# SandroMartens/DBGSOM

Measured on NVIDIA B200. Metric: training samples/sec/epoch, higher is better.
Workload: dtype f16 tensor cores (tcgen05) + f64 re-score / f64 update / f64 smoothing

## Files before the change

dbgsom_b200/csrc/bmu_tc.cu:

```cuda
#include <cuda.h>

#include <cstdio>
#include <cstdlib>

#include "common.cuh"

namespace dbgsom {

namespace {

constexpr int BM = 128;
constexpr int BK = 64;
constexpr int UMMA_K = 16;
constexpr int A_TILE_BYTES = BM * BK * 2;
constexpr int EPI_WARP0 = 4;
constexpr int EPI_SUBS = 4;
constexpr int EPI_WARPS = 4 * EPI_SUBS;
constexpr int EPI_THREADS = EPI_WARPS * 32;
constexpr int TC_THREADS = (EPI_WARP0 + EPI_WARPS) * 32;
constexpr int KSUB = 4;
constexpr int MAX_RES_KB = 4;
constexpr int kFlagMaxCols = 4096;
constexpr int kFlagChunkBytes = kFlagMaxCols / 32 * BM * 4;

// ... 190 lines not shown
}
__device__ __forceinline__ int4 lds_i4(uint32_t a) {
  int4 v;
  asm volatile("ld.shared.v4.s32 {%0,%1,%2,%3}, [%4];" : "=r"(v.x), "=r"(v.y), "=r"(v.z), "=r"(v.w) : "r"(a));
  return v;
}
__device__ __forceinline__ void sts_f1(uint32_t a, float v) { asm volatile("st.shared.f32 [%0], %1;" ::"r"(a), "f"(v) : "memory"); }
__device__ __forceinline__ void sts_i1(uint32_t a, int v) { asm volatile("st.shared.s32 [%0], %1;" ::"r"(a), "r"(v) : "memory"); }
__device__ __forceinline__ bool pair_after(float va, int ja, float vb, int jb) {
  return va > vb || (va == vb && ja > jb);
}

struct EpiConst {
  const int32_t* proto_of_col;
  uint32_t pstride, mpad;
  int any_order;
};
constexpr uint32_t kTabIdxOffset = 128 * 4 * 4 * 4;

__device__ __noinline__ float2 slow_offer(float s, int col, uint32_t val_addr, uint32_t const_addr) {
  const EpiConst* ec;
  {
    uint64_t g;
    asm volatile("cvta.shared.u64 %0, %1;" : "=l"(g) : "l"((uint64_t)const_addr));
    ec = reinterpret_cast<const EpiConst*>(g);
  }
  const uint32_t idx_addr = val_addr + kTabIdxOffset;
  const int j = ec->pstride ? (int)(((uint32_t)col * ec->pstride) % ec->mpad) : ec->proto_of_col[col];
  const float4 v4 = lds_f4(val_addr);
  const int4 j4 = lds_i4(idx_addr);
  float v0 = v4.x, v1 = v4.y, v2 = v4.z, v3 = v4.w;
  int c0 = j4.x, c1 = j4.y, c2 = j4.z, c3 = j4.w;
  int w = 0;
  float wv = v0;
  int wc = c0;
  if (pair_after(v1, c1, wv, wc)) { w = 1; wv = v1; wc = c1; }
  if (pair_after(v2, c2, wv, wc)) { w = 2; wv = v2; wc = c2; }
  if (pair_after(v3, c3, wv, wc)) { w = 3; wv = v3; wc = c3; }
  const bool replace = pair_after(wv, wc, s, j);
  const float out = replace ? wv : s;
  if (replace) {
    sts_f1(val_addr + 4 * w, s);
    sts_i1(idx_addr + 4 * w, j);
    if (w == 0) v0 = s;
    if (w == 1) v1 = s;
    if (w == 2) v2 = s;
    if (w == 3) v3 = s;
  }
  float g = fmaxf(fmaxf(v0, v1), fmaxf(v2, v3));
  if (!ec->any_order && g < 3.0e38f) g = nextafterf(g, __int_as_float(0x7f800000));
  return make_float2(g, out);
}

template <int NPASS, int BN, int RES_KB, int AKB, bool PAIRS = false, int EXTRA_BYTES = 0>
struct Cfg {
  static constexpr bool ATM = AKB > 0;
  static constexpr bool XRES = RES_KB > 0;
  static constexpr bool ASTREAM = !XRES && !ATM;
  static constexpr int NA = NPASS == 3 ? 2 : 1;
  static constexpr int B_TILE_BYTES = BN * BK * 2;
  static_assert(!PAIRS || ASTREAM, "PAIRS is the streamed form");
  static constexpr int STAGE_BYTES = NA * (PAIRS ? B_TILE_BYTES / 2 : B_TILE_BYTES) + (ASTREAM ? NA * A_TILE_BYTES : 0);
  static_assert(!ATM || (RES_KB == 0 && B_TILE_BYTES <= A_TILE_BYTES), "TMEM-resident A shares the ring: BN <= 128");
  static constexpr int A_COLS = AKB * NA * (BK / 2);
  static constexpr int NACC = ATM ? ((512 - A_COLS) / BN > 4 ? 4 : (512 - A_COLS) / BN) : (PAIRS && BN == 128 ? 4 : 2);
  static_assert(NACC >= 2, "need two accumulator buffers");
  static constexpr int RES_BYTES = RES_KB * NA * A_TILE_BYTES;
  static constexpr int RING_BYTES = BM * EPI_SUBS * KSUB * 8 + BM * 4 + BM * EPI_SUBS * 16;
  static constexpr int MISC_BYTES = 1024;
  static constexpr int WN_SMEM_FLOATS = ATM ? 4096 : 0;
  static constexpr int WN_BYTES = WN_SMEM_FLOATS * 4;
  static constexpr int SMEM_BUDGET = 227 * 1024 - 1024;
  static constexpr int STAGE_UNIT = ATM ? (STAGE_BYTES > A_TILE_BYTES ? STAGE_BYTES : A_TILE_BYTES) : STAGE_BYTES;
  static constexpr int STAGES_RAW = (SMEM_BUDGET - RES_BYTES - RING_BYTES - MISC_BYTES - WN_BYTES - EXTRA_BYTES) / STAGE_UNIT;
  static constexpr int STAGES = STAGES_RAW > (ATM ? 12 : 8) ? (ATM ? 12 : 8) : STAGES_RAW;
  static constexpr int RING_STAGE_BYTES = STAGES * STAGE_UNIT;
  static constexpr int SMEM_BYTES = RES_BYTES + RING_STAGE_BYTES + RING_BYTES + MISC_BYTES + WN_BYTES + EXTRA_BYTES + 1024;
  static constexpr int TMEM_COLS = ATM ? 512 : NACC * BN;
  static_assert(STAGES >= 2, "not enough shared memory for a pipeline");
};

struct Barriers {
  uint64_t full[16], empty[16];
  uint64_t a_full, a_empty;
  uint64_t tmem_full[4], tmem_empty[4];
  uint32_t tmem_base;
  EpiConst epi;
};

constexpr float kTileBoundFloor = 0.125f;
template <int NPASS, int NB, int BN, int RES_KB, int AKB, int CL, bool PAIR = false, int SEL = 0, bool TB = false,
          int SGT = 0>
__global__ void __launch_bounds__(TC_THREADS, 1)
    bmu_cand_tensor_kernel(const __grid_constant__ CUtensorMap map_xh, const __grid_constant__ CUtensorMap map_xl,
                           const __grid_constant__ CUtensorMap map_wh, const __grid_constant__ CUtensorMap map_wl,
                           const __grid_constant__ CUtensorMap map_wb, const float* __restrict__ bias_scale,
                           int64_t N, int KB, int NT, const float* __restrict__ wnorm,
                           const int32_t* __restrict__ proto_of_col, int pstride, int ties_any,
                           const float* __restrict__ xnorm16,
                           const float* __restrict__ wmax, float bound_coef, float acc_coef,
                           int32_t* __restrict__ idx_out, int32_t* __restrict__ cand_idx,
                           uint8_t* __restrict__ cand_count, const int32_t* __restrict__ row_perm,
                           unsigned long long* __restrict__ tile_mask,
                           int fg_shift, unsigned long long* __restrict__ sel_stats,
                           const float* __restrict__ tile_bound) {
  static_assert(!TB || (NB == 1 && SEL == 0 && BN % 128 == 0), "tile bounds: classic one-winner search, 128-column granules");
  using C = Cfg<NPASS, BN, RES_KB, AKB, PAIR && AKB == 0 && RES_KB == 0, SEL == 1 ? kFlagChunkBytes : 0>;
  static_assert(SEL == 0 || (PAIR && AKB > 0 && NB == 1 && NPASS == (SEL == 1 ? 1 : 3)),
                "selective search: CTA pairs, sample tile in tensor memory, one winner");
  constexpr bool ATM = C::ATM;
  static_assert(!PAIR || (CL == 2 && (ATM || C::ASTREAM)), "the CTA-pair form needs a cluster of two; sample tile in tensor memory or streamed");
  constexpr int B_PART_BYTES = PAIR ? C::B_TILE_BYTES / 2 : C::B_TILE_BYTES;
  constexpr bool SEGM = PAIR && C::ASTREAM && BN == 128;
  constexpr int SEG = 4;
  constexpr bool SEGT = SGT > 0;
  static_assert(!SEGT || (PAIR && C::ASTREAM && BN == 256 && C::NACC == 2 && SEL == 0), "tensor-memory sums: streamed pair form, 256 columns");
  static_assert(!SEGM || BN / 32 == EPI_SUBS, "segmented accumulation: one chunk per epilogue warp and tile");
  constexpr bool PAIR_ATM = PAIR && ATM;
  constexpr int SLOT_BYTES = PAIR_ATM ? A_TILE_BYTES : C::STAGE_BYTES;
  constexpr int NSLOT = PAIR_ATM ? (C::RING_STAGE_BYTES / A_TILE_BYTES > 16 ? 16 : C::RING_STAGE_BYTES / A_TILE_BYTES)
                                 : C::STAGES;
  static_assert(!PAIR_ATM || C::NA * B_PART_BYTES <= SLOT_BYTES, "a prototype k-block of the pair form must fit a slot");
  constexpr int NACC = C::NACC;
  constexpr bool XRES = C::XRES;
  constexpr bool ASTREAM = C::ASTREAM;
  extern __shared__ uint8_t smem_raw[];
  uint8_t* smem = reinterpret_cast<uint8_t*>((reinterpret_cast<uintptr_t>(smem_raw) + 1023) & ~uintptr_t(1023));
  uint8_t* res_a = smem;
  uint8_t* stages = smem + C::RES_BYTES;
  float* wn_smem = reinterpret_cast<float*>(stages + C::RING_STAGE_BYTES);
  uint8_t* ring = stages + C::RING_STAGE_BYTES + C::WN_BYTES;
  Barriers* bars = reinterpret_cast<Barriers*>(ring + C::RING_BYTES);
  float* chunk_min = reinterpret_cast<float*>(ring + C::RING_BYTES + C::MISC_BYTES);
  float* tab_val = reinterpret_cast<float*>(ring);
  int* tab_idx = reinterpret_cast<int*>(ring + BM * EPI_SUBS * KSUB * 4);
  float* row_min = reinterpret_cast<float*>(ring + BM * EPI_SUBS * KSUB * 8);
  float4* sub_state = reinterpret_cast<float4*>(ring + BM * EPI_SUBS * KSUB * 8 + BM * 4);

  const int warp = threadIdx.x >> 5;
  const int lane = threadIdx.x & 31;
  const int64_t n_row_tiles = ceil_div<int64_t>(N, BM);
  const uint32_t cl_rank = CL > 1 ? cluster_ctarank() : 0u;
  const int64_t n_clusters = gridDim.x / CL;
  const int64_t cluster_id = blockIdx.x / CL;
  const int64_t n_iters = ceil_div<int64_t>(n_row_tiles, n_clusters * CL);
  constexpr uint16_t cl_mask = (uint16_t)((1u << CL) - 1u);
  auto tile_of = [&](int64_t it) { return (it * n_clusters + cluster_id) * CL + cl_rank; };
  const int64_t n_pairs = ceil_div<int64_t>(n_row_tiles, 2);
  auto pair_of = [&](int64_t it) { return it * n_clusters + cluster_id; };
  auto sel_mask = [&](int64_t it) -> unsigned long long {
    const int64_t pr = pair_of(it);
    return (SEL == 2 && pr < n_pairs) ? tile_mask[pr] : 0ull;
  };

  if (warp == 0 && lane == 0) {
    tma_prefetch_desc(&map_xh);
    tma_prefetch_desc(&map_wh);
    if (NPASS == 3) {
      tma_prefetch_desc(&map_xl);
      tma_prefetch_desc(&map_wl);
    }
  }
  if (warp == 1 && lane == 0) {
    for (int s = 0; s < NSLOT; ++s) {
      mbar_init(&bars->full[s], PAIR ? 2 : 1);
      mbar_init(&bars->empty[s], PAIR ? 1 : CL);
    }
    mbar_init(&bars->a_full, 1);
    mbar_init(&bars->a_empty, 1);
    for (int b = 0; b < NACC; ++b) {
      mbar_init(&bars->tmem_full[b], 1);
      mbar_init(&bars->tmem_empty[b], PAIR ? 2 * EPI_WARPS : EPI_THREADS);
    }
    asm volatile("fence.mbarrier_init.release.cluster;" ::: "memory");
  }
  if (warp == 2) {
    if (PAIR) {
      asm volatile("tcgen05.alloc.cta_group::2.sync.aligned.shared::cta.b32 [%0], %1;" ::"r"(smem_u32(&bars->tmem_base)),
                   "r"((uint32_t)C::TMEM_COLS)
                   : "memory");
      asm volatile("tcgen05.relinquish_alloc_permit.cta_group::2.sync.aligned;" ::: "memory");
    } else {
      asm volatile("tcgen05.alloc.cta_group::1.sync.aligned.shared::cta.b32 [%0], %1;" ::"r"(smem_u32(&bars->tmem_base)),
                   "r"((uint32_t)C::TMEM_COLS)
                   : "memory");
      asm volatile("tcgen05.relinquish_alloc_permit.cta_group::1.sync.aligned;" ::: "memory");
    }
  }
// ... 22 lines not shown
      unsigned long long pmask_next = SEL == 2 ? sel_mask(0) : 0ull;
      for (int64_t it = 0; it < n_iters; ++it) {
        const int row0 = (int)(tile_of(it) * BM);
        const unsigned long long pmask_it = pmask_next;
        if (SEL == 2) pmask_next = it + 1 < n_iters ? sel_mask(it + 1) : 0ull;
        if (XRES) {
          mbar_wait(&bars->a_empty, a_phase ^ 1);
          mbar_expect_tx(&bars->a_full, (uint32_t)(KB * C::NA * A_TILE_BYTES));
          for (int kb = 0; kb < KB; ++kb) {
            tma_load_2d(res_a + (kb * C::NA + 0) * A_TILE_BYTES, &map_xh, &bars->a_full, kb * BK, row0);
            if (NPASS == 3) tma_load_2d(res_a + (kb * C::NA + 1) * A_TILE_BYTES, &map_xl, &bars->a_full, kb * BK, row0);
          }
          a_phase ^= 1;
        }
        if (ATM) {
          for (int kb = 0; kb < KB; ++kb) {
            if (PAIR) {
              for (int h = 0; h < C::NA; ++h) {
                mbar_wait(&bars->empty[stage], phase ^ 1);
                const uint32_t lead_full = mapa_u32(smem_u32(&bars->full[stage]), 0);
                if (cl_rank == 0) mbar_expect_tx(&bars->full[stage], (uint32_t)(2 * A_TILE_BYTES));
                else mbar_arrive_cluster(lead_full);
                tma_load_2d_pair(stages + stage * SLOT_BYTES, h == 0 ? &map_xh : &map_xl, lead_full, kb * BK, row0);
                if (++stage == NSLOT) {
                  stage = 0;
                  phase ^= 1;
                }
              }
              continue;
            }
            mbar_wait(&bars->empty[stage], phase ^ 1);
            uint8_t* st = stages + stage * C::STAGE_BYTES;
            mbar_expect_tx(&bars->full[stage], (uint32_t)(C::NA * A_TILE_BYTES));
            tma_load_2d(st, &map_xh, &bars->full[stage], kb * BK, row0);
            if (NPASS == 3) tma_load_2d(st + A_TILE_BYTES, &map_xl, &bars->full[stage], kb * BK, row0);
            if (++stage == C::STAGES) {
              stage = 0;
              phase ^= 1;
            }
          }
        }
        unsigned long long selm = pmask_it;
        const int n_sel = SEL == 2 ? __popcll(selm) : NT;
        if (SEL == 2 && cl_rank == 0 && pair_of(it) < n_pairs) {
          sel_tiles += (unsigned)n_sel;
          ++sel_pairs;
        }
        for (int ti = 0; ti < n_sel; ++ti) {
          int nt = ti;
          if (SEL == 2) {
            nt = __ffsll((long long)selm) - 1;
            selm &= selm - 1;
          }
          for (int kb = 0; kb < KB; ++kb) {
            mbar_wait(&bars->empty[stage], phase ^ 1);
            uint8_t* st = stages + stage * SLOT_BYTES;
            if (PAIR) {
              const uint32_t lead_full = mapa_u32(smem_u32(&bars->full[stage]), 0);
              if (cl_rank == 0) mbar_expect_tx(&bars->full[stage], (uint32_t)(2 * (C::NA * B_PART_BYTES + (ASTREAM ? C::NA * A_TILE_BYTES : 0))));
              else mbar_arrive_cluster(lead_full);
              const int prow = nt * BN + (int)cl_rank * (BN / 2);
              tma_load_2d_pair(st, &map_wh, lead_full, kb * BK, prow);
              if (NPASS == 3) tma_load_2d_pair(st + B_PART_BYTES, &map_wl, lead_full, kb * BK, prow);
              if (ASTREAM) {
                uint8_t* sa = st + C::NA * B_PART_BYTES;
                tma_load_2d_pair(sa, &map_xh, lead_full, kb * BK, row0);
                if (NPASS == 3) tma_load_2d_pair(sa + A_TILE_BYTES, &map_xl, lead_full, kb * BK, row0);
              }
              if (++stage == NSLOT) {
                stage = 0;
                phase ^= 1;
              }
              continue;
            }
            mbar_expect_tx(&bars->full[stage], (uint32_t)C::STAGE_BYTES);
            if (CL == 1) {
              tma_load_2d(st, &map_wh, &bars->full[stage], kb * BK, nt * BN);
              if (NPASS == 3) tma_load_2d(st + C::B_TILE_BYTES, &map_wl, &bars->full[stage], kb * BK, nt * BN);
            } else {
              const int part = C::B_TILE_BYTES / CL, prow = nt * BN + (int)cl_rank * (BN / CL);
              tma_load_2d_mc(st + cl_rank * part, &map_wh, &bars->full[stage], kb * BK, prow, cl_mask);
              if (NPASS == 3)
                tma_load_2d_mc(st + C::B_TILE_BYTES + cl_rank * part, &map_wl, &bars->full[stage], kb * BK, prow, cl_mask);
            }
            if (ASTREAM) {
              uint8_t* sa = st + C::NA * C::B_TILE_BYTES;
              tma_load_2d(sa, &map_xh, &bars->full[stage], kb * BK, row0);
              if (NPASS == 3) tma_load_2d(sa + A_TILE_BYTES, &map_xl, &bars->full[stage], kb * BK, row0);
            }
            if (++stage == C::STAGES) {
              stage = 0;
              phase ^= 1;
            }
          }
          if (PAIR && bias_mode) {
            mbar_wait(&bars->empty[stage], phase ^ 1);
            const uint32_t lead_full = mapa_u32(smem_u32(&bars->full[stage]), 0);
            if (cl_rank == 0) mbar_expect_tx(&bars->full[stage], (uint32_t)(2 * B_PART_BYTES));
            else mbar_arrive_cluster(lead_full);
            tma_load_2d_pair(stages + stage * SLOT_BYTES, &map_wb, lead_full, 0, nt * BN + (int)cl_rank * (BN / 2));
            if (++stage == NSLOT) {
              stage = 0;
              phase ^= 1;
            }
          }
        }
      }
      if (SEL == 2 && sel_stats != nullptr && sel_pairs) {
        atomicAdd(sel_stats + 0, sel_tiles);
        atomicAdd(sel_stats + 1, sel_pairs);
      }
    }
  } else if (warp == 1 && (!PAIR || cl_rank == 0)) {
    if (elect_one()) {
      constexpr uint32_t idesc = instr_desc_f16(PAIR ? 2 * BM : BM, BN);
      int stage = 0;
// ... 2 lines not shown
      unsigned long long mask_next = SEL == 2 ? sel_mask(0) : 0ull;
      for (int64_t it = 0; it < n_iters; ++it) {
        const unsigned long long mask_it = mask_next;
        if (SEL == 2) mask_next = it + 1 < n_iters ? sel_mask(it + 1) : 0ull;
        if (XRES) {
          mbar_wait(&bars->a_full, a_phase);
          a_phase ^= 1;
        }
        const uint32_t tmem_a = tmem_base + NACC * BN;
        if (ATM) {
          for (int kb = 0; kb < KB; ++kb) {
            if (PAIR) {
              for (int h = 0; h < C::NA; ++h) {
                mbar_wait(&bars->full[stage], phase);
                tc_fence_after();
                const uint32_t sa = smem_u32(stages + stage * SLOT_BYTES);
#pragma unroll
                for (int k = 0; k < BK / UMMA_K; ++k)
                  tc_cp_128x256b_pair(tmem_a + h * AKB * (BK / 2) + kb * (BK / 2) + k * 8,
                                      smem_desc_sw128(sa + k * UMMA_K * 2));
                tc_commit_pair(&bars->empty[stage], cl_mask);
                if (++stage == NSLOT) {
                  stage = 0;
                  phase ^= 1;
                }
              }
              continue;
            }
            mbar_wait(&bars->full[stage], phase);
            tc_fence_after();
            const uint32_t sa = smem_u32(stages + stage * C::STAGE_BYTES);
#pragma unroll
            for (int k = 0; k < BK / UMMA_K; ++k) {
              tc_cp_128x256b(tmem_a + kb * (BK / 2) + k * 8, smem_desc_sw128(sa + k * UMMA_K * 2));
              if (NPASS == 3)
                tc_cp_128x256b(tmem_a + AKB * (BK / 2) + kb * (BK / 2) + k * 8,
                               smem_desc_sw128(sa + A_TILE_BYTES + k * UMMA_K * 2));
            }
            if (CL == 1) tc_commit(&bars->empty[stage]); else tc_commit_mc(&bars->empty[stage], cl_mask);
            if (++stage == C::STAGES) {
              stage = 0;
              phase ^= 1;
            }
          }
        }
        const int n_sel = SEL == 2 ? __popcll(mask_it) : NT;
        for (int nt = 0; nt < n_sel; ++nt) {
          uint32_t tmem_d = tmem_base + acc * BN;
          if (!SEGM && !SEGT) {
            mbar_wait(&bars->tmem_empty[acc], acc_phase ^ 1);
            tc_fence_after();
          }
          uint32_t region = acc;
          for (int kb = 0; kb < KB; ++kb) {
            if (SEGM && kb % SEG == 0) {
              mbar_wait(&bars->tmem_empty[acc], acc_phase ^ 1);
              tc_fence_after();
              tmem_d = tmem_base + acc * BN;
            }
            if (SEGT && kb % (SEGT ? SGT : 1) == 0) {
              region = kb == 0 ? acc : acc ^ 1u;
              mbar_wait(&bars->tmem_empty[region], ((rph >> region) & 1u) ^ 1u);
              tc_fence_after();
              tmem_d = tmem_base + region * BN;
            }
            mbar_wait(&bars->full[stage], phase);
            tc_fence_after();
            uint8_t* st = stages + stage * SLOT_BYTES;
            const uint32_t b_hi = smem_u32(st);
            const uint32_t b_lo = b_hi + B_PART_BYTES;
            const uint32_t a_hi = XRES ? smem_u32(res_a + kb * C::NA * A_TILE_BYTES)
                                       : smem_u32(st + C::NA * B_PART_BYTES);
            const uint32_t a_lo = a_hi + A_TILE_BYTES;
#pragma unroll
            for (int k = 0; k < BK / UMMA_K; ++k) {
              const uint32_t koff = k * UMMA_K * 2;
              if (PAIR && ASTREAM) {
                tc_mma_f16_ss_pair(tmem_d, smem_desc_sw128(a_hi + koff), smem_desc_sw128(b_hi + koff), idesc,
                                   ((SEGM ? kb % SEG : SEGT ? kb % (SEGT ? SGT : 1) : kb) | k) != 0);
                if (NPASS == 3) {
                  tc_mma_f16_ss_pair(tmem_d, smem_desc_sw128(a_hi + koff), smem_desc_sw128(b_lo + koff), idesc, 1);
                  tc_mma_f16_ss_pair(tmem_d, smem_desc_sw128(a_lo + koff), smem_desc_sw128(b_hi + koff), idesc, 1);
                }
              } else if (PAIR) {
                const uint32_t ta_hi = tmem_a + kb * (BK / 2) + k * 8;
                const uint32_t ta_lo = ta_hi + AKB * (BK / 2);
                tc_mma_f16_ts_pair(tmem_d, ta_hi, smem_desc_sw128(b_hi + koff), idesc, (kb | k) != 0);
                if (NPASS == 3) {
                  tc_mma_f16_ts_pair(tmem_d, ta_hi, smem_desc_sw128(b_lo + koff), idesc, 1);
                  tc_mma_f16_ts_pair(tmem_d, ta_lo, smem_desc_sw128(b_hi + koff), idesc, 1);
                }
              } else if (ATM) {
                const uint32_t ta_hi = tmem_a + kb * (BK / 2) + k * 8;
                const uint32_t ta_lo = ta_hi + AKB * (BK / 2);
                tc_mma_f16_ts(tmem_d, ta_hi, smem_desc_sw128(b_hi + koff), idesc, (kb | k) != 0);
                if (NPASS == 3) {
                  tc_mma_f16_ts(tmem_d, ta_hi, smem_desc_sw128(b_lo + koff), idesc, 1);
                  tc_mma_f16_ts(tmem_d, ta_lo, smem_desc_sw128(b_hi + koff), idesc, 1);
                }
              } else {
                tc_mma_f16(tmem_d, smem_desc_sw128(a_hi + koff), smem_desc_sw128(b_hi + koff), idesc, (kb | k) != 0);
                if (NPASS == 3) {
                  tc_mma_f16(tmem_d, smem_desc_sw128(a_hi + koff), smem_desc_sw128(b_lo + koff), idesc, 1);
                  tc_mma_f16(tmem_d, smem_desc_sw128(a_lo + koff), smem_desc_sw128(b_hi + koff), idesc, 1);
                }
              }
            }
            if (PAIR) tc_commit_pair(&bars->empty[stage], cl_mask);
            else if (CL == 1) tc_commit(&bars->empty[stage]); else tc_commit_mc(&bars->empty[stage], cl_mask);
            if (++stage == NSLOT) {
              stage = 0;
              phase ^= 1;
            }
            if (SEGT && (kb % (SEGT ? SGT : 1) == (SEGT ? SGT : 1) - 1 || kb == KB - 1)) {
              tc_commit_pair(&bars->tmem_full[region], cl_mask);
              rph ^= 1u << region;
            }
            if (SEGM && kb % SEG == SEG - 1 && kb != KB - 1) {
              tc_commit_pair(&bars->tmem_full[acc], cl_mask);
              if (++acc == NACC) {
                acc = 0;
                acc_phase ^= 1;
              }
            }
          }
          if (PAIR && bias_mode) {
            mbar_wait(&bars->full[stage], phase);
            tc_fence_after();
            tc_mma_f16_ss_pair(tmem_d, smem_desc_sw128(smem_u32(wn_smem)), smem_desc_sw128(smem_u32(stages + stage * SLOT_BYTES)),
                               idesc, 1);
            tc_commit_pair(&bars->empty[stage], cl_mask);
            if (++stage == NSLOT) {
              stage = 0;
              phase ^= 1;
            }
          }
          if (SEGT) {
          } else if (PAIR) tc_commit_pair(&bars->tmem_full[acc], cl_mask); else tc_commit(&bars->tmem_full[acc]);
          if (++acc == NACC) {
            acc = 0;
            acc_phase ^= 1;
          }
        }
        if (XRES) tc_commit(&bars->a_empty);
      }
    }
  } else if (warp >= EPI_WARP0) {
    const int quarter = warp & 3;
    const int sub = (warp - EPI_WARP0) >> 2;
    const int t = quarter * 32 + lane;
    const uint32_t lane_base = (uint32_t)(quarter * 32) << 16;
    static_assert(KSUB == 4 && BM * EPI_SUBS * KSUB * 4 == kTabIdxOffset, "slow_offer handles four-entry tables");
    const uint32_t my_val_addr = smem_u32(tab_val + (t * EPI_SUBS + sub) * KSUB);
    const uint32_t my_idx_addr = my_val_addr + kTabIdxOffset;
    const bool any_order = NB == 1 && ties_any != 0;
    if (threadIdx.x == EPI_WARP0 * 32) {
      bars->epi.proto_of_col = proto_of_col;
      bars->epi.pstride = (uint32_t)pstride;
      bars->epi.mpad = (uint32_t)(NT * BN);
      bars->epi.any_order = any_order ? 1 : 0;
    }
    const uint32_t epi_const_addr = smem_u32(&bars->epi);
    constexpr int CHUNKS = BN / 32;
    constexpr float kInf = 3.0e38f;
    if (sub == 0) row_min[t] = kInf;
    const int mpad = NT * BN;
    const bool wn_in_smem = !bias_mode && C::WN_SMEM_FLOATS > 0 && mpad <= C::WN_SMEM_FLOATS;
    if (wn_in_smem)
      for (int i = threadIdx.x - EPI_WARP0 * 32; i < mpad; i += EPI_THREADS) wn_smem[i] = wnorm[i];
    const float* wn_src = wn_in_smem ? wn_smem : wnorm;
    asm volatile("bar.sync 1, %0;" ::"n"(EPI_THREADS));
    uint32_t acc = 0, acc_phase = 0;
    uint32_t eph = 0;
    (void)eph;
    if constexpr (SEL == 1) {
      uint32_t* cta_mask = reinterpret_cast<uint32_t*>(sub_state);
      float* sub_min = reinterpret_cast<float*>(sub_state) + 4;
      if (threadIdx.x == EPI_WARP0 * 32) cta_mask[0] = cta_mask[1] = 0u;
      asm volatile("bar.sync 1, %0;" ::"n"(EPI_THREADS));
      const int n_chunks = NT * CHUNKS;
      for (int64_t it = 0; it < n_iters; ++it) {
        const int64_t row = tile_of(it) * BM + t;
        const bool valid = row < N;
        const int64_t orow = valid ? (row_perm ? (int64_t)row_perm[row] : row) : 0;
        const float tau = valid ? 2.f * tensor_score_bound(xnorm16[orow], wmax, bound_coef, acc_coef) : 0.f;
        float m1 = kInf;
        for (int nt = 0; nt < NT; ++nt) {
          mbar_wait(&bars->tmem_full[acc], acc_phase);
          tc_fence_after();
          const uint32_t tmem_acc = tmem_base + lane_base + acc * BN;
#pragma unroll 1
          for (int c = (sub - nt * CHUNKS) & (EPI_SUBS - 1); c < CHUNKS; c += EPI_SUBS) {
            uint32_t r[32];
            tmem_ld_32x32(tmem_acc + c * 32, r);
            float a1;
            if (bias_mode) {
              tmem_ld_wait();
              float gmx[8];
#pragma unroll
              for (int g = 0; g < 8; ++g)
                gmx[g] = fmaxf(fmaxf(__uint_as_float(r[4 * g + 0]), __uint_as_float(r[4 * g + 1])),
                               fmaxf(__uint_as_float(r[4 * g + 2]), __uint_as_float(r[4 * g + 3])));
              a1 = -2.f * fmaxf(fmaxf(fmaxf(gmx[0], gmx[1]), fmaxf(gmx[2], gmx[3])),
                                fmaxf(fmaxf(gmx[4], gmx[5]), fmaxf(gmx[6], gmx[7])));
            } else {
              const int col = nt * BN + c * 32;
              const float4* wn4 = reinterpret_cast<const float4*>(wn_src + col);
              float4 w4[8];
#pragma unroll
              for (int g = 0; g < 8; ++g) w4[g] = wn4[g];
              tmem_ld_wait();
              float gmn[8];
#pragma unroll
              for (int g = 0; g < 8; ++g) {
                const float s0 = fmaf(-2.f, __uint_as_float(r[4 * g + 0]), w4[g].x);
                const float s1 = fmaf(-2.f, __uint_as_float(r[4 * g + 1]), w4[g].y);
                const float s2 = fmaf(-2.f, __uint_as_float(r[4 * g + 2]), w4[g].z);
                const float s3 = fmaf(-2.f, __uint_as_float(r[4 * g + 3]), w4[g].w);
// ... 11 lines not shown
          if (++acc == NACC) {
            acc = 0;
            acc_phase ^= 1;
          }
        }
        sub_min[t * EPI_SUBS + sub] = m1;
        asm volatile("bar.sync 1, %0;" ::"n"(EPI_THREADS));
        const float4 sm4 = *reinterpret_cast<const float4*>(sub_min + t * EPI_SUBS);
        const float thr = fminf(fminf(sm4.x, sm4.y), fminf(sm4.z, sm4.w)) + tau;
        uint32_t mlo = 0u, mhi = 0u;
        if (valid) {
          for (int ch = sub; ch < n_chunks; ch += EPI_SUBS) {
            const uint32_t bit = (uint32_t)(ch * 32) >> fg_shift;
            const uint32_t inb = chunk_min[ch * BM + t] <= thr ? 1u : 0u;
            mlo |= bit < 32u ? inb << bit : 0u;
            mhi |= bit >= 32u ? inb << (bit - 32u) : 0u;
          }
        }
        mlo = __reduce_or_sync(kFullMask, mlo);
        mhi = __reduce_or_sync(kFullMask, mhi);
        if (lane == 0) {
          if (mlo) atomicOr(&cta_mask[0], mlo);
          if (mhi) atomicOr(&cta_mask[1], mhi);
        }
        asm volatile("bar.sync 1, %0;" ::"n"(EPI_THREADS));
        if (threadIdx.x == EPI_WARP0 * 32) {
          const unsigned long long m64 = (unsigned long long)cta_mask[0] | ((unsigned long long)cta_mask[1] << 32);
          const int64_t pr = pair_of(it);
          if (m64 && pr < n_pairs) atomicOr(tile_mask + pr, m64);
          cta_mask[0] = cta_mask[1] = 0u;
        }
        asm volatile("bar.sync 1, %0;" ::"n"(EPI_THREADS));
      }
    } else {
    auto fetch_orow = [&](int64_t it_) -> int64_t {
      const int64_t r_ = it_ < n_iters ? tile_of(it_) * BM + t : N;
      return r_ < N ? (row_perm ? (int64_t)row_perm[r_] : r_) : -1;
    };
    auto fetch_mask = [&](int64_t it_) -> unsigned long long { return it_ < n_iters ? sel_mask(it_) : 0ull; };
    int64_t orow_n1 = fetch_orow(0);
    int64_t orow_n2 = fetch_orow(1);
    float xn_n1 = orow_n1 >= 0 ? xnorm16[orow_n1] : 0.f;
    unsigned long long mask_n1 = fetch_mask(0);
    for (int64_t it = 0; it < n_iters; ++it) {
      const int64_t row = tile_of(it) * BM + t;
      const int64_t orow = orow_n1 >= 0 ? orow_n1 : 0;
      const float tau = row < N ? 2.f * tensor_score_bound(xn_n1, wmax, bound_coef, acc_coef) : 0.f;
      const float xn_row = row < N ? xn_n1 : 0.f;
      unsigned long long selm = mask_n1;
      orow_n1 = orow_n2;
      xn_n1 = orow_n1 >= 0 ? xnorm16[orow_n1] : 0.f;
      orow_n2 = fetch_orow(it + 2);
      mask_n1 = fetch_mask(it + 1);
      float m1 = kInf, m2 = kInf, thr = kInf, evicted = __int_as_float(0x7f800000);
      float gate = __int_as_float(0x7f800000);
      asm volatile("st.shared.v4.f32 [%0], {%1,%1,%1,%1};" ::"r"(my_val_addr), "f"(gate) : "memory");
      asm volatile("st.shared.v4.s32 [%0], {%1,%1,%1,%1};" ::"r"(my_idx_addr), "r"(0x7fffffff) : "memory");
      const int n_sel = SEL == 2 ? __popcll(selm) : NT;
      for (int ti = 0; ti < n_sel; ++ti) {
        int nt = ti;
        if (SEL == 2) {
          nt = __ffsll((long long)selm) - 1;
          selm &= selm - 1;
        }
        float kb = 0.f;
        if (TB) {
          const float* tb = tile_bound + 2 * (nt * (BN / 128));
          float um = tb[0], wm = tb[1];
#pragma unroll
          for (int q = 1; q < BN / 128; ++q) {
            um = fmaxf(um, tb[2 * q]);
            wm = fmaxf(wm, tb[2 * q + 1]);
          }
          um = fmaxf(um, kTileBoundFloor * wmax[0]);
          wm = fmaxf(wm, kTileBoundFloor * wmax[2]);
          const float xw = xn_row * um;
          kb = xw * bound_coef + acc_coef * (xw + wm);
        }
        if constexpr (SEGT) {
          const uint32_t R = acc, Q = acc ^ 1u;
          mbar_wait(&bars->tmem_full[R], (eph >> R) & 1u);
          eph ^= 1u << R;
          const int nseg = (KB + SGT - 1) / SGT;
          for (int sg = 1; sg < nseg; ++sg) {
            mbar_wait(&bars->tmem_full[Q], (eph >> Q) & 1u);
            eph ^= 1u << Q;
            tc_fence_after();
#pragma unroll 1
            for (int c = (sub - ti * CHUNKS) & (EPI_SUBS - 1); c < CHUNKS; c += EPI_SUBS) {
              uint32_t p0[16], q0[16], p1[16], q1[16];
              const uint32_t pa = tmem_base + lane_base + Q * BN + c * 32, qa = tmem_base + lane_base + R * BN + c * 32;
              tmem_ld_32x16(pa, p0);
              tmem_ld_32x16(qa, q0);
              tmem_ld_32x16(pa + 16, p1);
              tmem_ld_32x16(qa + 16, q1);
              tmem_ld_wait();
              if (c + EPI_SUBS >= CHUNKS) {
                tc_fence_before();
                __syncwarp();
                if (lane == 0) mbar_arrive_cluster(mapa_u32(smem_u32(&bars->tmem_empty[Q]), 0));
              }
#pragma unroll
              for (int e = 0; e < 16; ++e) {
                q0[e] = __float_as_uint(__uint_as_float(q0[e]) + __uint_as_float(p0[e]));
                q1[e] = __float_as_uint(__uint_as_float(q1[e]) + __uint_as_float(p1[e]));
              }
              tmem_st_32x16(qa, q0);
              tmem_st_32x16(qa + 16, q1);
            }
            tmem_st_wait();
// ... 13 lines not shown
              if (seg > 0) {
                mbar_wait(&bars->tmem_full[acc], acc_phase);
                tc_fence_after();
              }
              tmem_ld_32x32(tmem_base + lane_base + acc * BN + c * 32, r);
              tmem_ld_wait();
#pragma unroll
              for (int e = 0; e < 32; ++e) sum[e] = seg == 0 ? __uint_as_float(r[e]) : sum[e] + __uint_as_float(r[e]);
              if (seg < nseg - 1) {
                tc_fence_before();
                __syncwarp();
                if (lane == 0) mbar_arrive_cluster(mapa_u32(smem_u32(&bars->tmem_empty[acc]), 0));
                if (++acc == NACC) {
                  acc = 0;
                  acc_phase ^= 1;
                }
              }
            }
#pragma unroll
            for (int e = 0; e < 32; ++e) r[e] = __float_as_uint(sum[e]);
          } else {
            tmem_ld_32x32(tmem_acc + c * 32, r);
          }
          const int col = nt * BN + c * 32;
          const float4* wn4 = reinterpret_cast<const float4*>(wn_src + col);
          float4 w4[8];
          if (bias_mode) {
#pragma unroll
            for (int g = 0; g < 8; ++g) w4[g] = make_float4(0.f, 0.f, 0.f, 0.f);
          } else {
#pragma unroll
            for (int g = 0; g < 8; ++g) w4[g] = wn4[g];
          }
          tmem_ld_wait();
          float a1 = kInf, a2 = kInf;
          float gm[8];
#pragma unroll
          for (int g = 0; g < 8; ++g) {
            const float s0 = fmaf(-2.f, __uint_as_float(r[4 * g + 0]), w4[g].x);
            const float s1 = fmaf(-2.f, __uint_as_float(r[4 * g + 1]), w4[g].y);
            const float s2 = fmaf(-2.f, __uint_as_float(r[4 * g + 2]), w4[g].z);
            const float s3 = fmaf(-2.f, __uint_as_float(r[4 * g + 3]), w4[g].w);
            gm[g] = fminf(fminf(s0, s1), fminf(s2, s3));
            if (NB == 2) {
              a2 = fminf(a2, fmaxf(a1, s0)); a1 = fminf(a1, s0);
              a2 = fminf(a2, fmaxf(a1, s1)); a1 = fminf(a1, s1);
              a2 = fminf(a2, fmaxf(a1, s2)); a1 = fminf(a1, s2);
              a2 = fminf(a2, fmaxf(a1, s3)); a1 = fminf(a1, s3);
            }
          }
          if (NB == 1) a1 = fminf(fminf(fminf(gm[0], gm[1]), fminf(gm[2], gm[3])), fminf(fminf(gm[4], gm[5]), fminf(gm[6], gm[7])));
          if (TB) {
            const float v = a1 + kb;
            const float sh = row_min[t];
            if (v < sh) row_min[t] = v;
            m2 = fminf(m2, fmaxf(m1, v));
            m1 = fminf(m1, v);
            thr = fminf(m1, sh) + kb;
          } else if (NB == 1) {
            const float sh = row_min[t];
            if (a1 < sh) row_min[t] = a1;
            m1 = fminf(m1, fminf(a1, sh));
            thr = m1 + tau;
          } else {
            m2 = fminf(fmaxf(m1, a1), fminf(m2, a2));
            m1 = fminf(m1, a1);
            thr = m2 < 1.0e38f ? m2 + tau : kInf;
          }
          if (a1 <= thr) {
            if (a1 - kb >= gate) {
              evicted = fminf(evicted, a1 - kb);
            } else {
              uint32_t inb = 0;
#pragma unroll
              for (int g = 0; g < 8; ++g) {
                if (gm[g] <= thr) {
                  inb |= (fmaf(-2.f, __uint_as_float(r[4 * g + 0]), w4[g].x) <= thr ? 1u : 0u) << (4 * g + 0);
                  inb |= (fmaf(-2.f, __uint_as_float(r[4 * g + 1]), w4[g].y) <= thr ? 1u : 0u) << (4 * g + 1);
                  inb |= (fmaf(-2.f, __uint_as_float(r[4 * g + 2]), w4[g].z) <= thr ? 1u : 0u) << (4 * g + 2);
                  inb |= (fmaf(-2.f, __uint_as_float(r[4 * g + 3]), w4[g].w) <= thr ? 1u : 0u) << (4 * g + 3);
                }
              }
              if ((inb & (inb - 1)) == 0) {
                if (inb) {
                  const float2 o = slow_offer(a1 - kb, col + __ffs(inb) - 1, my_val_addr, epi_const_addr);
                  gate = o.x;
                  evicted = fminf(evicted, o.y);
                }
              } else {
                float sc[32];
                uint32_t need = 0;
#pragma unroll
                for (int g = 0; g < 8; ++g) {
                  sc[4 * g + 0] = fmaf(-2.f, __uint_as_float(r[4 * g + 0]), w4[g].x);
                  sc[4 * g + 1] = fmaf(-2.f, __uint_as_float(r[4 * g + 1]), w4[g].y);
                  sc[4 * g + 2] = fmaf(-2.f, __uint_as_float(r[4 * g + 2]), w4[g].z);
                  sc[4 * g + 3] = fmaf(-2.f, __uint_as_float(r[4 * g + 3]), w4[g].w);
#pragma unroll
                  for (int e = 0; e < 4; ++e) {
                    const float se = sc[4 * g + e];
                    const bool in = se <= thr, out = se - kb >= gate;
                    evicted = fminf(evicted, in && out ? se - kb : __int_as_float(0x7f800000));
                    need |= (in && !out ? 1u : 0u) << (4 * g + e);
                  }
                }
#pragma unroll 1
                while (need) {
                  const int e = __ffs(need) - 1;
                  need &= need - 1;
                  const float se = sc[e] - kb;
                  if (se >= gate) {
                    evicted = fminf(evicted, se);
                  } else {
                    const float2 o = slow_offer(se, col + e, my_val_addr, epi_const_addr);
                    gate = o.x;
                    evicted = fminf(evicted, o.y);
                  }
                }
              }
            }
          }
        }
        tc_fence_before();
        if (PAIR) {
          __syncwarp();
          if (lane == 0) mbar_arrive_cluster(mapa_u32(smem_u32(&bars->tmem_empty[acc]), 0));
        } else {
          mbar_arrive(&bars->tmem_empty[acc]);
        }
        if (++acc == NACC) {
          acc = 0;
          acc_phase ^= 1;
        }
      }
      sub_state[t * EPI_SUBS + sub] = make_float4(m1, m2, evicted, 0.f);
      asm volatile("bar.sync 1, %0;" ::"n"(EPI_THREADS));
      if (sub == 0) {
        float g1 = kInf, g2 = kInf, ev = __int_as_float(0x7f800000);
#pragma unroll
        for (int q = 0; q < EPI_SUBS; ++q) {
          const float4 st = sub_state[t * EPI_SUBS + q];
          if (NB == 2 || TB) g2 = fminf(fmaxf(g1, st.x), fminf(g2, st.y));
          g1 = fminf(g1, st.x);
          ev = fminf(ev, st.z);
        }
        const float gm = NB == 1 ? g1 : g2;
        const float gthr = gm < 1.0e38f ? (TB ? gm : gm + tau) : kInf;
        float v[EPI_SUBS * KSUB];
        int jx[EPI_SUBS * KSUB];
#pragma unroll
        for (int q = 0; q < EPI_SUBS; ++q) {
          const float4 v4 = lds_f4(smem_u32(tab_val + (t * EPI_SUBS + q) * KSUB));
          const int4 j4 = lds_i4(smem_u32(tab_idx + (t * EPI_SUBS + q) * KSUB));
          v[4 * q + 0] = v4.x; v[4 * q + 1] = v4.y; v[4 * q + 2] = v4.z; v[4 * q + 3] = v4.w;
          jx[4 * q + 0] = j4.x; jx[4 * q + 1] = j4.y; jx[4 * q + 2] = j4.z; jx[4 * q + 3] = j4.w;
        }
        int cnt = 0, best = -1;
        float bv = __int_as_float(0x7f800000), sv = __int_as_float(0x7f800000);
        bool overflow = ev <= gthr;
#pragma unroll
        for (int i = 0; i < EPI_SUBS * KSUB; ++i) {
          const bool in = v[i] <= gthr;
          const bool first = in && (v[i] < bv || (v[i] == bv && jx[i] < best));
          const bool second = in && !first && v[i] < sv;
          cnt += in ? 1 : 0;
          sv = first ? bv : (second ? v[i] : sv);
          bv = first ? v[i] : bv;
          best = first ? jx[i] : best;
        }
        if (cnt > kMaxCand) overflow = true;
        if (row < N) {
          int32_t* slots = cand_idx + orow * kMaxCand;
          if (overflow) {
            slots[0] = __float_as_int(fmaxf((TB ? (g2 < 1.0e38f ? g2 : __int_as_float(0x7f800000)) : sv) - bv, 0.f));
          } else if (cnt == 1) {
            slots[0] = best;
          } else {
            int w = 0;
#pragma unroll
            for (int i = 0; i < EPI_SUBS * KSUB; ++i)
              if (v[i] <= gthr) slots[w++] = jx[i];
          }
          cand_count[orow] = (uint8_t)(overflow ? DBGSOM_CAND_OVERFLOW : cnt);
          idx_out[orow * NB] = best;
        }
        row_min[t] = kInf;
      }
      asm volatile("bar.sync 1, %0;" ::"n"(EPI_THREADS));
    }
    }
  }

  tc_fence_before();
  __syncthreads();
  if (CL > 1) cluster_sync_all();
  if (warp == 2) {
    tc_fence_after();
    if (PAIR)
      asm volatile("tcgen05.dealloc.cta_group::2.sync.aligned.b32 %0, %1;" ::"r"(tmem_base), "r"((uint32_t)C::TMEM_COLS)
                   : "memory");
    else
      asm volatile("tcgen05.dealloc.cta_group::1.sync.aligned.b32 %0, %1;" ::"r"(tmem_base), "r"((uint32_t)C::TMEM_COLS)
                   : "memory");
  }
}

typedef CUresult (*EncodeTiledFn)(CUtensorMap*, CUtensorMapDataType, cuuint32_t, void*, const cuuint64_t*,
                                  const cuuint64_t*, const cuuint32_t*, const cuuint32_t*, CUtensorMapInterleave,
                                  CUtensorMapSwizzle, CUtensorMapL2promotion, CUtensorMapFloatOOBfill);

EncodeTiledFn encode_tiled_fn() {
  static EncodeTiledFn fn = nullptr;
  static bool tried = false;
  if (!tried) {
    tried = true;
    void* p = nullptr;
    cudaDriverEntryPointQueryResult q;
    if (cudaGetDriverEntryPoint("cuTensorMapEncodeTiled", &p, cudaEnableDefault, &q) == cudaSuccess &&
        q == cudaDriverEntryPointSuccess)
      fn = reinterpret_cast<EncodeTiledFn>(p);
  }
  return fn;
}

int make_map(CUtensorMap* map, const uint16_t* base, int64_t rows, int64_t ld, int box_rows) {
  EncodeTiledFn fn = encode_tiled_fn();
  if (!fn) return DBGSOM_E_DRIVER;
  const cuuint64_t dims[2] = {(cuuint64_t)ld, (cuuint64_t)rows};
  const cuuint64_t strides[1] = {(cuuint64_t)ld * 2};
  const cuuint32_t box[2] = {(cuuint32_t)BK, (cuuint32_t)box_rows};
  const cuuint32_t elem[2] = {1, 1};
  const CUresult r = fn(map, CU_TENSOR_MAP_DATA_TYPE_FLOAT16, 2, const_cast<uint16_t*>(base), dims, strides, box, elem,
                        CU_TENSOR_MAP_INTERLEAVE_NONE, CU_TENSOR_MAP_SWIZZLE_128B, CU_TENSOR_MAP_L2_PROMOTION_L2_256B,
                        CU_TENSOR_MAP_FLOAT_OOB_FILL_NONE);
  return r == CUDA_SUCCESS ? DBGSOM_OK : DBGSOM_E_DRIVER;
}

int sm_count() {
  static int n = 0;
  if (n == 0) {
    int dev = 0;
    cudaGetDevice(&dev);
    cudaDeviceGetAttribute(&n, cudaDevAttrMultiProcessorCount, dev);
    if (n <= 0) n = 148;
  }
  return n;
}

template <int NPASS, int NB, int BN, int RES_KB, int AKB, int CL, bool PAIR = false, int SEL = 0, bool TB = false, int SGT = 0>
int launch_cfg_cl(const dbgsom_bmu_args& a, const BmuWorkspace& ws, cudaStream_t s) {
  using C = Cfg<NPASS, BN, RES_KB, AKB, PAIR && AKB == 0 && RES_KB == 0, SEL == 1 ? kFlagChunkBytes : 0>;
  CUtensorMap mxh, mxl, mwh, mwl;
  int rc = make_map(&mxh, a.d_X16_hi, a.N, a.ld16, BM);
  if (rc) return rc;
  rc = make_map(&mwh, a.d_W16_hi, a.Mpad, a.ld16, BN / CL);
  if (rc) return rc;
  if (NPASS == 3) {
    rc = make_map(&mxl, a.d_X16_lo, a.N, a.ld16, BM);
    if (rc) return rc;
    rc = make_map(&mwl, a.d_W16_lo, a.Mpad, a.ld16, BN / CL);
    if (rc) return rc;
  } else {
    mxl = mxh;
    mwl = mwh;
  }
  CUtensorMap mwb = mwh;
  const bool with_bias = (SEL == 0 || (SEL == 1 && AKB <= 2)) && PAIR && C::ATM && a.d_Wb16 != nullptr && a.d_bias_scale != nullptr;
  if (with_bias) {
    rc = make_map(&mwb, a.d_Wb16, a.Mpad, BK, BN / CL);
    if (rc) return rc;
  }
  if (with_bias && getenv("DBGSOM_TC_VERBOSE")) {
    static bool said = false;
    if (!said) {
      said = true;
      float e = -1.f;
      cudaMemcpy(&e, a.d_bias_scale, sizeof(float), cudaMemcpyDeviceToHost);
      fprintf(stderr, "dbgsom: K1 takes wnorm through the bias k-step, E = %g\n", e);
    }
  }
  auto kern = bmu_cand_tensor_kernel<NPASS, NB, BN, RES_KB, AKB, CL, PAIR, SEL, TB, SGT>;
  DBGSOM_CUDA_TRY(cudaFuncSetAttribute(kern, cudaFuncAttributeMaxDynamicSharedMemorySize, C::SMEM_BYTES));
  const int KB = (int)(a.ld16 / BK);
  const int NT = a.Mpad / BN;
  int64_t grid = round_up<int64_t>(ceil_div<int64_t>(a.N, BM), CL);
  int64_t max_grid = sm_count() / CL * CL;
  cudaLaunchConfig_t cfg = {};
  cfg.gridDim = dim3((unsigned)max_grid);
  cfg.blockDim = dim3(TC_THREADS);
  cfg.dynamicSmemBytes = C::SMEM_BYTES;
  cfg.stream = s;
  cudaLaunchAttribute attr[1];
  attr[0].id = cudaLaunchAttributeClusterDimension;
  attr[0].val.clusterDim.x = CL;
  attr[0].val.clusterDim.y = 1;
  attr[0].val.clusterDim.z = 1;
  cfg.attrs = attr;
  cfg.numAttrs = CL > 1 ? 1 : 0;
  if (CL > 1) {
    static int max_clusters = 0;
    if (max_clusters == 0) {
      DBGSOM_CUDA_TRY(cudaFuncSetAttribute(kern, cudaFuncAttributeNonPortableClusterSizeAllowed, 0));
      if (cudaOccupancyMaxActiveClusters(&max_clusters, kern, &cfg) != cudaSuccess || max_clusters <= 0) {
        (void)cudaGetLastError();
// ... 162 lines not shown
```

Before: 323.1 million.

## Double-buffer epilogue reduction tables and pack two k-blocks per pair-form stage

For the selective search (SEL==2), the epilogue's per-row candidate tables, row minima and sub-state are double-buffered and alternate by iteration. This removes the trailing named barrier, so the final reduction of one row tile overlaps with the start of the next, and the reducing sub-warp moves to the last one. In the pair form with the sample tile in tensor memory, the producer and MMA issuer also handle two prototype k-blocks per ring slot when they fit, which halves barrier round-trips. The cost is more shared memory for the ring tables, which can reduce pipeline stages, plus a risk of races from dropping the barrier.

```diff
diff --git a/dbgsom_b200/csrc/bmu_tc.cu b/dbgsom_b200/csrc/bmu_tc.cu
--- a/dbgsom_b200/csrc/bmu_tc.cu
+++ b/dbgsom_b200/csrc/bmu_tc.cu
@@ -266,7 +266,7 @@
   return make_float2(g, out);
 }
 
-template <int NPASS, int BN, int RES_KB, int AKB, bool PAIRS = false, int EXTRA_BYTES = 0>
+template <int NPASS, int BN, int RES_KB, int AKB, bool PAIRS = false, int EXTRA_BYTES = 0, int NRING = 1>
 struct Cfg {
   static constexpr bool ATM = AKB > 0;
   static constexpr bool XRES = RES_KB > 0;
@@ -280,7 +280,8 @@
   static constexpr int NACC = ATM ? ((512 - A_COLS) / BN > 4 ? 4 : (512 - A_COLS) / BN) : (PAIRS && BN == 128 ? 4 : 2);
   static_assert(NACC >= 2, "need two accumulator buffers");
   static constexpr int RES_BYTES = RES_KB * NA * A_TILE_BYTES;
-  static constexpr int RING_BYTES = BM * EPI_SUBS * KSUB * 8 + BM * 4 + BM * EPI_SUBS * 16;
+  static constexpr int RING_ONE_BYTES = BM * EPI_SUBS * KSUB * 8 + BM * 4 + BM * EPI_SUBS * 16;
+  static constexpr int RING_BYTES = NRING * RING_ONE_BYTES;
   static constexpr int MISC_BYTES = 1024;
   static constexpr int WN_SMEM_FLOATS = ATM ? 4096 : 0;
   static constexpr int WN_BYTES = WN_SMEM_FLOATS * 4;
@@ -319,7 +320,7 @@
                            int fg_shift, unsigned long long* __restrict__ sel_stats,
                            const float* __restrict__ tile_bound) {
   static_assert(!TB || (NB == 1 && SEL == 0 && BN % 128 == 0), "tile bounds: classic one-winner search, 128-column granules");
-  using C = Cfg<NPASS, BN, RES_KB, AKB, PAIR && AKB == 0 && RES_KB == 0, SEL == 1 ? kFlagChunkBytes : 0>;
+  using C = Cfg<NPASS, BN, RES_KB, AKB, PAIR && AKB == 0 && RES_KB == 0, SEL == 1 ? kFlagChunkBytes : 0, SEL == 2 ? 2 : 1>;
   static_assert(SEL == 0 || (PAIR && AKB > 0 && NB == 1 && NPASS == (SEL == 1 ? 1 : 3)),
                 "selective search: CTA pairs, sample tile in tensor memory, one winner");
   constexpr bool ATM = C::ATM;
@@ -335,6 +336,7 @@
   constexpr int NSLOT = PAIR_ATM ? (C::RING_STAGE_BYTES / A_TILE_BYTES > 16 ? 16 : C::RING_STAGE_BYTES / A_TILE_BYTES)
                                  : C::STAGES;
   static_assert(!PAIR_ATM || C::NA * B_PART_BYTES <= SLOT_BYTES, "a prototype k-block of the pair form must fit a slot");
+  constexpr int KPS = PAIR_ATM && 2 * C::NA * B_PART_BYTES <= SLOT_BYTES ? 2 : 1;
   constexpr int NACC = C::NACC;
   constexpr bool XRES = C::XRES;
   constexpr bool ASTREAM = C::ASTREAM;
@@ -347,7 +349,6 @@
   Barriers* bars = reinterpret_cast<Barriers*>(ring + C::RING_BYTES);
   float* chunk_min = reinterpret_cast<float*>(ring + C::RING_BYTES + C::MISC_BYTES);
   float* tab_val = reinterpret_cast<float*>(ring);
-  int* tab_idx = reinterpret_cast<int*>(ring + BM * EPI_SUBS * KSUB * 4);
   float* row_min = reinterpret_cast<float*>(ring + BM * EPI_SUBS * KSUB * 8);
   float4* sub_state = reinterpret_cast<float4*>(ring + BM * EPI_SUBS * KSUB * 8 + BM * 4);
 
@@ -476,16 +477,20 @@
             nt = __ffsll((long long)selm) - 1;
             selm &= selm - 1;
           }
-          for (int kb = 0; kb < KB; ++kb) {
+          for (int kb = 0; kb < KB; kb += KPS) {
             mbar_wait(&bars->empty[stage], phase ^ 1);
             uint8_t* st = stages + stage * SLOT_BYTES;
             if (PAIR) {
+              const int nk = KB - kb < KPS ? KB - kb : KPS;
               const uint32_t lead_full = mapa_u32(smem_u32(&bars->full[stage]), 0);
-              if (cl_rank == 0) mbar_expect_tx(&bars->full[stage], (uint32_t)(2 * (C::NA * B_PART_BYTES + (ASTREAM ? C::NA * A_TILE_BYTES : 0))));
+              if (cl_rank == 0) mbar_expect_tx(&bars->full[stage], (uint32_t)(2 * (nk * C::NA * B_PART_BYTES + (ASTREAM ? C::NA * A_TILE_BYTES : 0))));
               else mbar_arrive_cluster(lead_full);
               const int prow = nt * BN + (int)cl_rank * (BN / 2);
-              tma_load_2d_pair(st, &map_wh, lead_full, kb * BK, prow);
-              if (NPASS == 3) tma_load_2d_pair(st + B_PART_BYTES, &map_wl, lead_full, kb * BK, prow);
+              for (int j = 0; j < nk; ++j) {
+                uint8_t* sj = st + j * C::NA * B_PART_BYTES;
+                tma_load_2d_pair(sj, &map_wh, lead_full, (kb + j) * BK, prow);
+                if (NPASS == 3) tma_load_2d_pair(sj + B_PART_BYTES, &map_wl, lead_full, (kb + j) * BK, prow);
+              }
               if (ASTREAM) {
                 uint8_t* sa = st + C::NA * B_PART_BYTES;
                 tma_load_2d_pair(sa, &map_xh, lead_full, kb * BK, row0);
@@ -594,7 +599,7 @@
             tc_fence_after();
           }
           uint32_t region = acc;
-          for (int kb = 0; kb < KB; ++kb) {
+          for (int kb = 0; kb < KB; kb += KPS) {
             if (SEGM && kb % SEG == 0) {
               mbar_wait(&bars->tmem_empty[acc], acc_phase ^ 1);
               tc_fence_after();
@@ -614,37 +619,42 @@
             const uint32_t a_hi = XRES ? smem_u32(res_a + kb * C::NA * A_TILE_BYTES)
                                        : smem_u32(st + C::NA * B_PART_BYTES);
             const uint32_t a_lo = a_hi + A_TILE_BYTES;
-#pragma unroll
-            for (int k = 0; k < BK / UMMA_K; ++k) {
-              const uint32_t koff = k * UMMA_K * 2;
-              if (PAIR && ASTREAM) {
-                tc_mma_f16_ss_pair(tmem_d, smem_desc_sw128(a_hi + koff), smem_desc_sw128(b_hi + koff), idesc,
-                                   ((SEGM ? kb % SEG : SEGT ? kb % (SEGT ? SGT : 1) : kb) | k) != 0);
-                if (NPASS == 3) {
-                  tc_mma_f16_ss_pair(tmem_d, smem_desc_sw128(a_hi + koff), smem_desc_sw128(b_lo + koff), idesc, 1);
-                  tc_mma_f16_ss_pair(tmem_d, smem_desc_sw128(a_lo + koff), smem_desc_sw128(b_hi + koff), idesc, 1);
-                }
-              } else if (PAIR) {
-                const uint32_t ta_hi = tmem_a + kb * (BK / 2) + k * 8;
-                const uint32_t ta_lo = ta_hi + AKB * (BK / 2);
-                tc_mma_f16_ts_pair(tmem_d, ta_hi, smem_desc_sw128(b_hi + koff), idesc, (kb | k) != 0);
-                if (NPASS == 3) {
-                  tc_mma_f16_ts_pair(tmem_d, ta_hi, smem_desc_sw128(b_lo + koff), idesc, 1);
-                  tc_mma_f16_ts_pair(tmem_d, ta_lo, smem_desc_sw128(b_hi + koff), idesc, 1);
-                }
-              } else if (ATM) {
-                const uint32_t ta_hi = tmem_a + kb * (BK / 2) + k * 8;
-                const uint32_t ta_lo = ta_hi + AKB * (BK / 2);
-                tc_mma_f16_ts(tmem_d, ta_hi, smem_desc_sw128(b_hi + koff), idesc, (kb | k) != 0);
-                if (NPASS == 3) {
-                  tc_mma_f16_ts(tmem_d, ta_hi, smem_desc_sw128(b_lo + koff), idesc, 1);
-                  tc_mma_f16_ts(tmem_d, ta_lo, smem_desc_sw128(b_hi + koff), idesc, 1);
-                }
-              } else {
-                tc_mma_f16(tmem_d, smem_desc_sw128(a_hi + koff), smem_desc_sw128(b_hi + koff), idesc, (kb | k) != 0);
-                if (NPASS == 3) {
-                  tc_mma_f16(tmem_d, smem_desc_sw128(a_hi + koff), smem_desc_sw128(b_lo + koff), idesc, 1);
-                  tc_mma_f16(tmem_d, smem_desc_sw128(a_lo + koff), smem_desc_sw128(b_hi + koff), idesc, 1);
+            const int nk = KB - kb < KPS ? KB - kb : KPS;
+            for (int j = 0; j < nk; ++j) {
+              const int kbj = kb + j;
+              const uint32_t bh = b_hi + j * C::NA * B_PART_BYTES, bl = b_lo + j * C::NA * B_PART_BYTES;
+#pragma unroll
+              for (int k = 0; k < BK / UMMA_K; ++k) {
+                const uint32_t koff = k * UMMA_K * 2;
+                if (PAIR && ASTREAM) {
+                  tc_mma_f16_ss_pair(tmem_d, smem_desc_sw128(a_hi + koff), smem_desc_sw128(b_hi + koff), idesc,
+                                     ((SEGM ? kb % SEG : SEGT ? kb % (SEGT ? SGT : 1) : kb) | k) != 0);
+                  if (NPASS == 3) {
+                    tc_mma_f16_ss_pair(tmem_d, smem_desc_sw128(a_hi + koff), smem_desc_sw128(b_lo + koff), idesc, 1);
+                    tc_mma_f16_ss_pair(tmem_d, smem_desc_sw128(a_lo + koff), smem_desc_sw128(b_hi + koff), idesc, 1);
+                  }
+                } else if (PAIR) {
+                  const uint32_t ta_hi = tmem_a + kbj * (BK / 2) + k * 8;
+                  const uint32_t ta_lo = ta_hi + AKB * (BK / 2);
+                  tc_mma_f16_ts_pair(tmem_d, ta_hi, smem_desc_sw128(bh + koff), idesc, (kbj | k) != 0);
+                  if (NPASS == 3) {
+                    tc_mma_f16_ts_pair(tmem_d, ta_hi, smem_desc_sw128(bl + koff), idesc, 1);
+                    tc_mma_f16_ts_pair(tmem_d, ta_lo, smem_desc_sw128(bh + koff), idesc, 1);
+                  }
+                } else if (ATM) {
+                  const uint32_t ta_hi = tmem_a + kb * (BK / 2) + k * 8;
+                  const uint32_t ta_lo = ta_hi + AKB * (BK / 2);
+                  tc_mma_f16_ts(tmem_d, ta_hi, smem_desc_sw128(b_hi + koff), idesc, (kb | k) != 0);
+                  if (NPASS == 3) {
+                    tc_mma_f16_ts(tmem_d, ta_hi, smem_desc_sw128(b_lo + koff), idesc, 1);
+                    tc_mma_f16_ts(tmem_d, ta_lo, smem_desc_sw128(b_hi + koff), idesc, 1);
+                  }
+                } else {
+                  tc_mma_f16(tmem_d, smem_desc_sw128(a_hi + koff), smem_desc_sw128(b_hi + koff), idesc, (kb | k) != 0);
+                  if (NPASS == 3) {
+                    tc_mma_f16(tmem_d, smem_desc_sw128(a_hi + koff), smem_desc_sw128(b_lo + koff), idesc, 1);
+                    tc_mma_f16(tmem_d, smem_desc_sw128(a_lo + koff), smem_desc_sw128(b_hi + koff), idesc, 1);
+                  }
                 }
               }
             }
@@ -694,7 +704,6 @@
     const uint32_t lane_base = (uint32_t)(quarter * 32) << 16;
     static_assert(KSUB == 4 && BM * EPI_SUBS * KSUB * 4 == kTabIdxOffset, "slow_offer handles four-entry tables");
     const uint32_t my_val_addr = smem_u32(tab_val + (t * EPI_SUBS + sub) * KSUB);
-    const uint32_t my_idx_addr = my_val_addr + kTabIdxOffset;
     const bool any_order = NB == 1 && ties_any != 0;
     if (threadIdx.x == EPI_WARP0 * 32) {
       bars->epi.proto_of_col = proto_of_col;
@@ -705,7 +714,8 @@
     const uint32_t epi_const_addr = smem_u32(&bars->epi);
     constexpr int CHUNKS = BN / 32;
     constexpr float kInf = 3.0e38f;
-    if (sub == 0) row_min[t] = kInf;
+    if (sub == 0)
+      for (int b = 0; b < C::RING_BYTES / C::RING_ONE_BYTES; ++b) row_min[b * (C::RING_ONE_BYTES / 4) + t] = kInf;
     const int mpad = NT * BN;
     const bool wn_in_smem = !bias_mode && C::WN_SMEM_FLOATS > 0 && mpad <= C::WN_SMEM_FLOATS;
     if (wn_in_smem)
@@ -823,10 +833,13 @@
       xn_n1 = orow_n1 >= 0 ? xnorm16[orow_n1] : 0.f;
       orow_n2 = fetch_orow(it + 2);
       mask_n1 = fetch_mask(it + 1);
+      const uint32_t rb_off = SEL == 2 ? (uint32_t)(it & 1) * C::RING_ONE_BYTES : 0u;
+      const uint32_t val_addr = my_val_addr + rb_off;
+      float* rmin = reinterpret_cast<float*>(reinterpret_cast<uint8_t*>(row_min) + rb_off);
       float m1 = kInf, m2 = kInf, thr = kInf, evicted = __int_as_float(0x7f800000);
       float gate = __int_as_float(0x7f800000);
-      asm volatile("st.shared.v4.f32 [%0], {%1,%1,%1,%1};" ::"r"(my_val_addr), "f"(gate) : "memory");
-      asm volatile("st.shared.v4.s32 [%0], {%1,%1,%1,%1};" ::"r"(my_idx_addr), "r"(0x7fffffff) : "memory");
+      asm volatile("st.shared.v4.f32 [%0], {%1,%1,%1,%1};" ::"r"(val_addr), "f"(gate) : "memory");
+      asm volatile("st.shared.v4.s32 [%0], {%1,%1,%1,%1};" ::"r"(val_addr + kTabIdxOffset), "r"(0x7fffffff) : "memory");
       const int n_sel = SEL == 2 ? __popcll(selm) : NT;
       for (int ti = 0; ti < n_sel; ++ti) {
         int nt = ti;
@@ -946,14 +959,14 @@
           if (NB == 1) a1 = fminf(fminf(fminf(gm[0], gm[1]), fminf(gm[2], gm[3])), fminf(fminf(gm[4], gm[5]), fminf(gm[6], gm[7])));
           if (TB) {
             const float v = a1 + kb;
-            const float sh = row_min[t];
-            if (v < sh) row_min[t] = v;
+            const float sh = rmin[t];
+            if (v < sh) rmin[t] = v;
             m2 = fminf(m2, fmaxf(m1, v));
             m1 = fminf(m1, v);
             thr = fminf(m1, sh) + kb;
           } else if (NB == 1) {
-            const float sh = row_min[t];
-            if (a1 < sh) row_min[t] = a1;
+            const float sh = rmin[t];
+            if (a1 < sh) rmin[t] = a1;
             m1 = fminf(m1, fminf(a1, sh));
             thr = m1 + tau;
           } else {
@@ -977,7 +990,7 @@
               }
               if ((inb & (inb - 1)) == 0) {
                 if (inb) {
-                  const float2 o = slow_offer(a1 - kb, col + __ffs(inb) - 1, my_val_addr, epi_const_addr);
+                  const float2 o = slow_offer(a1 - kb, col + __ffs(inb) - 1, val_addr, epi_const_addr);
                   gate = o.x;
                   evicted = fminf(evicted, o.y);
                 }
@@ -1006,7 +1019,7 @@
                   if (se >= gate) {
                     evicted = fminf(evicted, se);
                   } else {
-                    const float2 o = slow_offer(se, col + e, my_val_addr, epi_const_addr);
+                    const float2 o = slow_offer(se, col + e, val_addr, epi_const_addr);
                     gate = o.x;
                     evicted = fminf(evicted, o.y);
                   }
@@ -1027,13 +1040,15 @@
           acc_phase ^= 1;
         }
       }
-      sub_state[t * EPI_SUBS + sub] = make_float4(m1, m2, evicted, 0.f);
+      const uint32_t val_base = smem_u32(tab_val) + rb_off;
+      float4* sst = reinterpret_cast<float4*>(reinterpret_cast<uint8_t*>(sub_state) + rb_off);
+      sst[t * EPI_SUBS + sub] = make_float4(m1, m2, evicted, 0.f);
       asm volatile("bar.sync 1, %0;" ::"n"(EPI_THREADS));
-      if (sub == 0) {
+      if (sub == EPI_SUBS - 1) {
         float g1 = kInf, g2 = kInf, ev = __int_as_float(0x7f800000);
 #pragma unroll
         for (int q = 0; q < EPI_SUBS; ++q) {
-          const float4 st = sub_state[t * EPI_SUBS + q];
+          const float4 st = sst[t * EPI_SUBS + q];
           if (NB == 2 || TB) g2 = fminf(fmaxf(g1, st.x), fminf(g2, st.y));
           g1 = fminf(g1, st.x);
           ev = fminf(ev, st.z);
@@ -1044,8 +1059,8 @@
         int jx[EPI_SUBS * KSUB];
 #pragma unroll
         for (int q = 0; q < EPI_SUBS; ++q) {
-          const float4 v4 = lds_f4(smem_u32(tab_val + (t * EPI_SUBS + q) * KSUB));
-          const int4 j4 = lds_i4(smem_u32(tab_idx + (t * EPI_SUBS + q) * KSUB));
+          const float4 v4 = lds_f4(val_base + 4 * ((t * EPI_SUBS + q) * KSUB));
+          const int4 j4 = lds_i4(val_base + kTabIdxOffset + 4 * ((t * EPI_SUBS + q) * KSUB));
           v[4 * q + 0] = v4.x; v[4 * q + 1] = v4.y; v[4 * q + 2] = v4.z; v[4 * q + 3] = v4.w;
           jx[4 * q + 0] = j4.x; jx[4 * q + 1] = j4.y; jx[4 * q + 2] = j4.z; jx[4 * q + 3] = j4.w;
         }
@@ -1078,9 +1093,9 @@
           cand_count[orow] = (uint8_t)(overflow ? DBGSOM_CAND_OVERFLOW : cnt);
           idx_out[orow * NB] = best;
         }
-        row_min[t] = kInf;
+        rmin[t] = kInf;
       }
-      asm volatile("bar.sync 1, %0;" ::"n"(EPI_THREADS));
+      if (SEL != 2) asm volatile("bar.sync 1, %0;" ::"n"(EPI_THREADS));
     }
     }
   }
@@ -1143,7 +1158,7 @@
 
 template <int NPASS, int NB, int BN, int RES_KB, int AKB, int CL, bool PAIR = false, int SEL = 0, bool TB = false, int SGT = 0>
 int launch_cfg_cl(const dbgsom_bmu_args& a, const BmuWorkspace& ws, cudaStream_t s) {
-  using C = Cfg<NPASS, BN, RES_KB, AKB, PAIR && AKB == 0 && RES_KB == 0, SEL == 1 ? kFlagChunkBytes : 0>;
+  using C = Cfg<NPASS, BN, RES_KB, AKB, PAIR && AKB == 0 && RES_KB == 0, SEL == 1 ? kFlagChunkBytes : 0, SEL == 2 ? 2 : 1>;
   CUtensorMap mxh, mxl, mwh, mwl;
   int rc = make_map(&mxh, a.d_X16_hi, a.N, a.ld16, BM);
   if (rc) return rc;
```

Result: slower. 315.0 million, median of 6 (-2.5%).
